# JuliaLinearAlgebra/AlgebraicMultigrid.jl

Hardware: AMD Instinct MI355X
Metric: V-cycle unknowns/sec + fine-level SpMV GB/s (% HBM peak), 3-D Poisson 256^3 (higher is better)
Workload: dtype f64

## Files before the change

algebraicmultigrid.jl_amd/_libs.py:

```python
import ctypes as C
import os

_HERE = os.path.dirname(os.path.abspath(__file__))
SETUP_SO = os.path.join(_HERE, "libamgsetup.so")
HIP_SO = os.path.join(_HERE, "libamghip.so")
HIP_F32_SO = os.path.join(_HERE, "libamghip_f32.so")

i32p = C.POINTER(C.c_int32)
f64p = C.POINTER(C.c_double)
i64 = C.c_int64
vp = C.c_void_p


class AMGError(RuntimeError):
    pass


class amgs_options(C.Structure):
    _fields_ = [("theta", C.c_double), ("max_levels", C.c_int32), ("max_coarse", C.c_int32),
                ("hermitian", C.c_int32), ("sa_omega", C.c_double), ("sa_improve_iters", C.c_int32),
                ("sa_B_is_vector", C.c_int32)]


class amgh_smoother_t(C.Structure):
# ... 141 lines not shown
    L.amgh_dev_upload.argtypes = [C.c_int, vp, vp, i64]
    L.amgh_dev_download.argtypes = [C.c_int, vp, vp, i64]
    L.amgh_dev_sync.argtypes = [C.c_int]
    L.amgh_stream.restype = vp
    L.amgh_stream.argtypes = [vp]
    L.amgh_timer_begin.argtypes = [vp]
    L.amgh_timer_end.argtypes = [vp, C.POINTER(C.c_double)]
    L.amgh_bench_op.argtypes = [vp, C.c_int, C.c_int, C.c_int, C.c_int, C.POINTER(C.c_double)]
    L.amgh_debug_chain_timing.argtypes = [C.c_int, vp]
    L.amgh_debug_merged_sweep_host.argtypes = [i64, i64, vp, vp, vp, C.c_int, C.c_int, C.c_double, vp, vp]
    L.amgh_debug_bw_poll_giveups.argtypes = [vp, C.c_int]
    L.amgh_debug_bw_mode.argtypes = [vp, C.c_int]
    L.amgh_debug_bw_dict.argtypes = [vp, C.c_int]
    L.amgh_debug_bw_late.argtypes = [vp, C.c_int]
    L.amgh_debug_coded_ops.argtypes = [vp, C.c_int]
    L.amgh_debug_bw_sweep_host.argtypes = [i64, vp, vp, vp, C.c_int, C.c_int, C.c_double, vp, vp, vp]
    L.amgh_debug_bw_dict_sweep_host.argtypes = [i64, vp, vp, vp, C.c_int, C.c_int, vp, vp, vp]
    L.amgh_debug_set_tunable.argtypes = [C.c_char_p, C.c_int]
    L.amgh_debug_get_tunable.argtypes = [C.c_char_p, C.POINTER(C.c_int)]
    L.amgh_profile_enable.argtypes = [vp, C.c_int]
    L.amgh_profile_read.argtypes = [vp, vp, C.c_int]
    L.amgh_set_use_graph.argtypes = [vp, C.c_int]


def _bind_dist(L):
    i64p = C.POINTER(i64)
    L.amgh_dist_rccl_available.argtypes = []
    L.amgh_dist_unique_id.argtypes = [vp]
    L.amgh_dist_create_rccl.argtypes = [C.POINTER(vp), C.c_int, C.c_int, C.c_int, vp]
    L.amgh_local_group_create.argtypes = [C.POINTER(vp), C.c_int]
# ... 101 lines not shown
```

algebraicmultigrid.jl_amd/csrc/hip/amghip.hip:

```cpp
#include "amghip_internal.hpp"
#include "gs_schedule.hpp"
#include "csr_ops.hpp"
#include "chebyshev.hpp"
#include "gmres_kernels.hpp"
#include "pcg_block_kernels.hpp"
#include "dist_pcg_kernels.hpp"

namespace {

constexpr int64_t kGraphAutoRows = 65536;

struct Level {
  int64_t n = 0, nc = 0;
  amgh_csr A, S, P, R;
  bool has_S = false;
  amgh_smoother_t pre{}, post{};
  real *res = nullptr, *cx = nullptr, *cb = nullptr, *tmp = nullptr;
  real* cheb_d = nullptr;
  ChebSide cheb[2];
  const ChebSide& cheb_of(const amgh_smoother_t& s) const { return &s == &post ? cheb[1] : cheb[0]; }
  real* il = nullptr;
  amgh_csr* smat() { return has_S ? &S : &A; }
  amgh_csr Pp, Rp;
  bool lo_ok = false;
  real* lo_val = nullptr;
  CodedCols lo_cc;
  bool r_stream = false, p_stream = false;
  bool lo_want = false;
  bool coarse_lo = false;
};

}

struct amgh_handle {
  int device = 0;
  int nrhs = 1;
  hipStream_t stream = nullptr;
  hipStream_t own_stream = nullptr;
  bool ext_stream = false;
  std::vector<Level*> levels;
// ... 202 lines not shown
  {
    ProfScope p(h, AMGH_T_PRESMOOTH, l);
    RC_TRY(smooth(h, L, L->pre, xc, xo, b, bs, xzero,  lo_io,  lo_io && !xzero,  lo));
  }
  if (lo) {
    Level* C = (L->coarse_lo && l + 1 < (int)h->levels.size()) ? h->levels[l + 1] : nullptr;
    GsSchedule* cg = C ? C->smat()->gs : nullptr;
    if (C && !(cg && C->lo_ok && cg->nblk == 0 && cg->cols_alloc >= bs)) return AMGH_ESTATE;
    const int64_t xs = g->xstride;
    {
      ProfScope p(h, AMGH_T_RESIDUAL, l);
      if (il_block(bs) && g_rhs_il >= 2)
        RC_TRY(resid_cols(bs, g->rowptr, g->col, L->lo_val ? L->lo_val : g->val, n, g->xp, xs, g->bp, n, L->res, n, h->stream, &L->lo_cc));
      else
        RC_TRY(raw_apply(M_RESID, g->rowptr, g->col, L->lo_val ? L->lo_val : g->val, n, g->xp, xs, g->bp, n, L->res, n,
                         h->stream, bs, &L->lo_cc));
    }
    {
      ProfScope p(h, AMGH_T_RESTRICT, l);
      if (L->il && il_block(bs) && !(L->r_stream && g_rhs_il == 1))
        RC_TRY(il_apply(bs, false, L->Rp.rowptr, L->Rp.col, L->Rp.val, nc, L->res, n, n, L->il, C ? cg->bp : L->cb, nc, h->stream, &L->Rp.cc));
      else
        RC_TRY(csr_apply(&L->Rp, M_SPMV, L->res, nullptr, C ? cg->bp : L->cb, h->stream, bs));
      if (C) cg->bp_cols = bs;
    }
    if (!C) RC_TRY(vec_fill(h, L->cx, nc * bs, 0.0));
    if (l == (int)h->levels.size() - 1) {
      ProfScope p(h, AMGH_T_COARSE, l + 1);
      for (int c = 0; c < bs; ++c) RC_TRY(coarse_solve(h, L->cx + c * nc, L->cb + c * nc));
    } else if (tail_here(h, l + 1, cyc) && (C != nullptr) == h->tail_lo) {
      ProfScope p(h, AMGH_T_COARSE, l + 1);
      RC_TRY(tail_apply(h, h->tail[cyc].M, nc, C ? cg->xp : L->cx, C ? cg->xstride : nc, C ? (const real*)cg->bp : (const real*)L->cb, nc, bs, false));
    } else {
      RC_TRY(cycle_next(h, l + 1, L->cx, L->cb, cyc, C != nullptr));
    }
    {
      ProfScope p(h, AMGH_T_PROLONG, l);
      if (L->il && il_block(bs) && !(L->p_stream && g_rhs_il == 1))
        RC_TRY(il_apply(bs, true, L->Pp.rowptr, L->Pp.col, L->Pp.val, n, C ? cg->xp : L->cx, nc, C ? cg->xstride : nc, L->il,
                        g->xp, xs, h->stream, &L->Pp.cc));
      else
        RC_TRY(raw_apply(M_ADD, L->Pp.rowptr, L->Pp.col, L->Pp.val, n, C ? cg->xp : L->cx, C ? cg->xstride : nc, nullptr, 0, g->xp,
                         xs, h->stream, bs, &L->Pp.cc));
    }
    {
      ProfScope p(h, AMGH_T_POSTSMOOTH, l);
      RC_TRY(smooth(h, L, L->post, xc, xo, b, bs, false, true, true,  lo_io));
    }
    return AMGH_OK;
  }
  {
    ProfScope p(h, AMGH_T_RESIDUAL, l);
    RC_TRY(csr_apply(&L->A, M_RESID, xc, b, L->res, h->stream, bs));
  }
  {
    ProfScope p(h, AMGH_T_RESTRICT, l);
    if (L->il && il_block(bs))
      RC_TRY(il_apply(bs, false, L->R.rowptr, L->R.col, L->R.val, nc, L->res, n, n, L->il, L->cb, nc, h->stream));
    else
      RC_TRY(csr_apply(&L->R, M_SPMV, L->res, nullptr, L->cb, h->stream, bs));
  }
  RC_TRY(vec_fill(h, L->cx, nc * bs, 0.0));
  if (l == (int)h->levels.size() - 1) {
    ProfScope p(h, AMGH_T_COARSE, l + 1);
    for (int c = 0; c < bs; ++c) RC_TRY(coarse_solve(h, L->cx + c * nc, L->cb + c * nc));
  } else if (tail_here(h, l + 1, cyc) && !h->tail_lo) {
    ProfScope p(h, AMGH_T_COARSE, l + 1);
    RC_TRY(tail_apply(h, h->tail[cyc].M, nc, L->cx, nc, L->cb, nc, bs, false));
  } else {
    RC_TRY(cycle_next(h, l + 1, L->cx, L->cb, cyc));
  }
  {
    ProfScope p(h, AMGH_T_PROLONG, l);
    if (L->il && il_block(bs))
      RC_TRY(il_apply(bs, true, L->P.rowptr, L->P.col, L->P.val, n, L->cx, nc, nc, L->il, xc, n, h->stream));
    else
      RC_TRY(csr_apply(&L->P, M_ADD, L->cx, nullptr, xc, h->stream, bs));
  }
  {
    ProfScope p(h, AMGH_T_POSTSMOOTH, l);
    const bool b_kept = (L->pre.kind == AMGH_SMOOTH_GS || L->pre.kind == AMGH_SMOOTH_SOR) && L->pre.iter > 0;
    RC_TRY(smooth(h, L, L->post, xc, xo, b, bs, false, b_kept));
  }
  if (xc != x) RC_TRY(vec_copy(h, x, xc, n * bs));
  return AMGH_OK;
}

int apply_once(amgh_t* h, real* x, const real* b, int cyc, bool xzero) {
  if (h->levels.empty()) {
    ProfScope p(h, AMGH_T_COARSE, 0);
    for (int c = 0; c < h->nrhs; ++c) RC_TRY(coarse_solve(h, x + c * h->ncoarse, b + c * h->ncoarse));
    return AMGH_OK;
// ... 479 lines not shown
  *hp = h;
  return AMGH_OK;
}

static void level_discard(Level* L);

void amgh_destroy(amgh_t* h) {
  if (!h) return;
  hipSetDevice(h->device);
  if (h->stream) hipStreamSynchronize(h->stream);
  if (h->pending_level) level_discard(h->pending_level);
  for (Level* L : h->levels) {
    csr_free(&L->A); csr_free(&L->S); csr_free(&L->P); csr_free(&L->R); csr_free(&L->Pp); csr_free(&L->Rp);
    hipFree(L->res); hipFree(L->cx); hipFree(L->cb); hipFree(L->tmp); hipFree(L->cheb_d); hipFree(L->lo_val); hipFree(L->il);
    L->lo_cc.free_dev();
    delete L;
  }
  csr_free(&h->finalA);
  hipFree(h->coarse_op); hipFree(h->res_final); hipFree(h->partial); hipFree(h->scal);
  hipFree(h->x0); hipFree(h->b0); hipFree(h->pc_r); hipFree(h->pc_c); hipFree(h->pc_u);
  hipFree(h->gm_V); hipFree(h->gm_t); hipFree(h->gm_sc); hipFree(h->gm_part); hipFree(h->gm_flags);
  hipFree(h->pb_r); hipFree(h->pb_c); hipFree(h->pb_u); hipFree(h->pb_part); hipFree(h->pb_sc); hipFree(h->pb_st);
  for (auto& t : h->tail) hipFree(t.M);
  for (auto& e : h->pending) { hipEventDestroy(e.a); hipEventDestroy(e.b); }
  for (auto& g : h->graphs) if (g.exec) hipGraphExecDestroy(g.exec);
  if (h->t0) hipEventDestroy(h->t0);
  if (h->t1) hipEventDestroy(h->t1);
  if (h->tb0) hipEventDestroy(h->tb0);
  if (h->tb1) hipEventDestroy(h->tb1);
  if (h->own_stream) hipStreamDestroy(h->own_stream);
  else if (h->stream) hipStreamDestroy(h->stream);
  delete h;
}

static void level_discard(Level* L) {
  csr_free(&L->A); csr_free(&L->S); csr_free(&L->P); csr_free(&L->R); csr_free(&L->Pp); csr_free(&L->Rp);
  hipFree(L->lo_val);
  L->lo_cc.free_dev();
  delete L;
}

namespace {
__global__ void perm_rowlen_kernel(const int32_t* rowptr, const int32_t* perm, int64_t n, int32_t* len) {
  const int64_t p = (int64_t)blockIdx.x * blockDim.x + threadIdx.x;
  if (p < n) len[p] = rowptr[perm[p] + 1] - rowptr[perm[p]];
}
__global__ void perm_rows_kernel(const int32_t* rowptr, const int32_t* col, const real* val, const int32_t* perm,
                                 const int32_t* new_rowptr, int64_t n, int32_t* ncol, real* nval) {
  const int ln = threadIdx.x % kWave;
  const int64_t waves = (int64_t)gridDim.x * (blockDim.x / kWave);
  for (int64_t p = (int64_t)blockIdx.x * (blockDim.x / kWave) + threadIdx.x / kWave; p < n; p += waves) {
    const int32_t src = rowptr[perm[p]], len = rowptr[perm[p] + 1] - src, dst = new_rowptr[p];
    for (int e = ln; e < len; e += kWave) { ncol[dst + e] = col[src + e]; nval[dst + e] = val[src + e]; }
// ... 465 lines not shown
      for (int v = 0; v < 2 && rc == AMGH_OK; ++v) {
        L->Rp.xcd_map = v == 1;
        rc = csr_apply(&L->Rp, M_SPMV, L->res, nullptr, L->cb, h->stream, 1);
        if (rc == AMGH_OK && hipEventRecord(h->t0, h->stream) != hipSuccess) rc = -1001;
        for (int r = 0; r < 4 && rc == AMGH_OK; ++r) rc = csr_apply(&L->Rp, M_SPMV, L->res, nullptr, L->cb, h->stream, 1);
        float t = 0.f;
        if (rc == AMGH_OK && (hipEventRecord(h->t1, h->stream) != hipSuccess || hipEventSynchronize(h->t1) != hipSuccess ||
                              hipEventElapsedTime(&t, h->t0, h->t1) != hipSuccess)) rc = -1001;
        ms[v] = t;
      }
      L->Rp.xcd_map = false;
      RC_TRY(rc);
      L->Rp.xcd_map = ms[1] < 0.93 * ms[0];
      if (getenv("AMGH_VERBOSE")) fprintf(stderr, "[amghip] n=%lld restriction: %.3f ms, XCD-contiguous %.3f ms -> %s\n", (long long)L->n, ms[0] / 4, ms[1] / 4, L->Rp.xcd_map ? "XCD-contiguous" : "plain");
    }
  if (gs_trim() && g_stream_code && g_trim_coded) {
    HIP_TRY(hipStreamSynchronize(h->stream));
    for (Level* L : h->levels) {
      for (amgh_csr* M : {&L->Rp, &L->Pp})
        if (M->cc.ccol && M->col && M->val) {
          hipFree(M->col); hipFree(M->val); M->col = nullptr; M->val = nullptr;
          M->bytes -= M->nnz * kEntB;
        }
      amgh_csr* S = L->smat();
      GsSchedule* g = S->gs;
      if (L->lo_cc.ccol && g && g->bw.on && g->bw.flow.on && !g->bw.rec && g->segs.empty() && !g->mf && !g->mb && g->col && g->val) {
        hipFree(g->col); hipFree(g->val); g->col = nullptr; g->val = nullptr;
        int64_t freed = g->nnz * kEntB;
        if (L->lo_val) { hipFree(L->lo_val); L->lo_val = nullptr; }
        g->csr_bytes -= freed; g->bytes -= freed; S->bytes -= freed;
// ... 354 lines not shown
  amgh_csr* op = nullptr;
  switch (which) {
    case AMGH_OP_A: op = &h->levels[level]->A; break;
    case AMGH_OP_P: op = &h->levels[level]->P; break;
    case AMGH_OP_R: op = &h->levels[level]->R; break;
  }
  return (op && op->rowptr) ? op : nullptr;
}

struct LoOp {
  const int32_t *rowptr = nullptr, *col = nullptr;
  const real* val = nullptr;
  int64_t nrows = 0, ncols = 0;
  const int32_t *row_perm = nullptr, *col_perm = nullptr;
  const CodedCols* cc = nullptr;
};
static bool level_lo_op(amgh_t* h, int level, int which, LoOp* o) {
  if (level < 0 || level >= (int)h->levels.size()) return false;
  Level* L = h->levels[level];
  GsSchedule* g = L->smat()->gs;
  if (!L->lo_ok || !g || !g->perm) return false;
  const int32_t* coarse_perm = nullptr;
  if (L->coarse_lo) {
    if (level + 1 >= (int)h->levels.size()) return false;
    GsSchedule* cg = h->levels[level + 1]->smat()->gs;
    if (!cg || !cg->perm) return false;
    coarse_perm = cg->perm;
  }
  switch (which) {
    case AMGH_OP_A:
      if ((int64_t)g->ncols != L->n) return false;
      *o = LoOp{g->rowptr, g->col, L->lo_val ? L->lo_val : g->val, L->n, L->n, g->perm, g->perm, &L->lo_cc};
      return g->rowptr != nullptr && !g->compacted;
    case AMGH_OP_P:
      *o = LoOp{L->Pp.rowptr, L->Pp.col, L->Pp.val, L->n, L->nc, g->perm, coarse_perm, &L->Pp.cc};
      return L->Pp.rowptr != nullptr;
    case AMGH_OP_R:
      *o = LoOp{L->Rp.rowptr, L->Rp.col, L->Rp.val, L->nc, L->n, coarse_perm, g->perm, &L->Rp.cc};
      return L->Rp.rowptr != nullptr;
  }
  return false;
}

static int level_apply(amgh_t* h, int level, int which, int mode, const real* x_d, const real* b_d, real* y_d) {
  if (amgh_csr* op = level_op(h, level, which)) return csr_apply(op, mode, x_d, b_d, y_d, h->stream);
  LoOp o;
  if (!level_lo_op(h, level, which, &o)) return AMGH_EINVAL;
  real *xi = nullptr, *yo = nullptr, *bi = nullptr;
  int rc = AMGH_OK;
  const real* xin = x_d;
  const real* bin = b_d;
  if (o.col_perm) {
    rc = dev_alloc(&xi, o.ncols);
// ... 272 lines not shown
      z ^= z >> 31;
      hx[i] = (real)(z >> 11) * (1.0 / 9007199254740992.0);
    }
    hipMemcpy(x, hx.data(), sizeof(real) * nx, hipMemcpyHostToDevice);
    hipMemcpy(b, hx.data(), sizeof(real) * nx, hipMemcpyHostToDevice);
    hipMemcpy(y, hx.data(), sizeof(real) * nx, hipMemcpyHostToDevice);
  }
  int rc = AMGH_OK;
  auto run = [&]() -> int {
    if (which == 4) {
      if (level >= (int)h->levels.size()) return AMGH_EINVAL;
      return level_smooth_enqueue(h, level, 0, y, b);
    }
    const int mode = (which == 3 || which == 5) ? M_RESID : M_SPMV;
    if (op) return csr_apply(op, mode, x, b, y, h->stream);
    return raw_apply(mode, lo.rowptr, lo.col, lo.val, lo.nrows, x, lo.ncols, b, lo.nrows, y, lo.nrows, h->stream, 1, lo.cc);
    if (which == 4) {
      if (level >= (int)h->levels.size()) return AMGH_EINVAL;
      return level_smooth_enqueue(h, level, 0, y, b);
    }
    return AMGH_EINVAL;
  };
  for (int i = 0; i < warmup && rc == AMGH_OK; ++i) rc = run();
  if (rc == AMGH_OK) {
    hipEventRecord(h->tb0, h->stream);
    for (int i = 0; i < reps && rc == AMGH_OK; ++i) rc = run();
    hipEventRecord(h->tb1, h->stream);
    hipEventSynchronize(h->tb1);
    float f = 0.f;
    hipEventElapsedTime(&f, h->tb0, h->tb1);
    *avg_ms = (double)f / reps;
// ... 308 lines not shown
  else if (!strcmp(name, "gs_bigslot")) *value = g_gs_bigslot;
  else if (!strcmp(name, "gs_super")) *value = g_gs_super;
  else if (!strcmp(name, "gs_block_pipe")) *value = g_gs_block_pipe;
  else return AMGH_EINVAL;
  return AMGH_OK;
}

int amgh_debug_set_perm_io(int on) {
  g_gs_flow_perm_io = on != 0;
  ++g_sched_epoch;
  return AMGH_OK;
}
int amgh_debug_get_perm_io(void) { return g_gs_flow_perm_io; }
int amgh_debug_perm_io_sweeps(int which) { return (which == 0 || which == 1) ? (int)(g_perm_io_sweeps[which] & 0x7fffffffu) : -1; }

int amgh_debug_chain_timing(int enable, unsigned long long* out8) {
  if (enable && !g_chain_tim) {
    HIP_TRY(hipMalloc((void**)&g_chain_tim, 8 * sizeof(unsigned long long)));
    HIP_TRY(hipMemset(g_chain_tim, 0, 8 * sizeof(unsigned long long)));
  }
  if (out8 && g_chain_tim) {
    HIP_TRY(hipDeviceSynchronize());
    HIP_TRY(hipMemcpy(out8, g_chain_tim, 8 * sizeof(unsigned long long), hipMemcpyDeviceToHost));
    HIP_TRY(hipMemset(g_chain_tim, 0, 8 * sizeof(unsigned long long)));
  }
  if (!enable && g_chain_tim) { hipFree(g_chain_tim); g_chain_tim = nullptr; }
  return AMGH_OK;
}

int amgh_profile_enable(amgh_t* h, int on) {
// ... 27 lines not shown
```

algebraicmultigrid.jl_amd/csrc/hip/amghip_internal.hpp:

```cpp
#pragma once
#include "amghip_kernels.hpp"
#include "gs_blocks.hpp"
#include "gs_flow.hpp"

#include <algorithm>
#include <chrono>
#include <cmath>
#include <cstdio>
#include <cstring>
#include <atomic>
#include <mutex>
#include <string>
#include <system_error>
#include <thread>
#include <utility>
#include <vector>

#include "../../../include/amghip.h"

using namespace amgh;

#define HIP_TRY(expr)                                   \
  do {                                                  \
    hipError_t e_ = (expr);                             \
// ... 286 lines not shown
    hipFree(rowmeta); hipFree(desc); hipFree(bp); hipFree(xp); hipFree(permx);
    d_lvl_ptr = rowptr = col = perm = dpos = nullptr; val = diag = bp = xp = nullptr; rowmeta = desc = nullptr; permx = nullptr;
  }
};

}

#include "dev_scan.hpp"

struct CodedCols {
  uint32_t* ccol = nullptr; real* vtab = nullptr; int n = 0;
  int64_t bytes = 0;
  void free_dev() { hipFree(ccol); hipFree(vtab); ccol = nullptr; vtab = nullptr; n = 0; bytes = 0; }
};

struct amgh_csr {
  CodedCols cc;
  bool cc_tried = false;
  bool xcd_map = false;
  int device = 0;
  int64_t nrows = 0, ncols = 0, nnz = 0;
  int32_t* rowptr = nullptr;
  int32_t* col = nullptr;
  real* val = nullptr;
  int32_t* dpos = nullptr;
  real* diag = nullptr;
  GsSchedule* gs = nullptr;
  int gs_nrhs_hint = 0;
  uint32_t pipe_epoch = 0; const void* pipe_rmbox = nullptr; int pipe_grid = 0;
  int64_t bytes = 0;
};

// ... 11 lines not shown
int g_gs_bw = 1;
int g_gs_bw_rows = 512;
int g_gs_bw_flow = 1;
int g_gs_bw_spin = 0;
int g_gs_bw_skip_pub = -1;
int g_gs_bw_nc = -1;
int g_gs_bw_nrhs = 1;
int g_gs_bw_chain = 1;
int g_stream_code = 1;
int g_trim_coded = 1;
int g_gs_bw_inorder = 0;
int g_gs_bw_dict = 1;
int g_gs_bw_relay = 3;
int g_gs_flow_xzero = 1;
int g_gs_flow_perm_io = 1;
unsigned int g_perm_io_sweeps[2] = {0, 0};
int g_gs_bw_two_min_rows = 200000;
int g_gs_sell = 1;
int g_gs_lean = -1;
int g_gs_ept = 0;
int g_gs_lpr = 0;
int g_gs_il = 1;
int g_pcg_fused = 1;
int g_tail_dense_rows = 6144;
int g_tail_dense = 1;
int g_gs_dense_blk = 4096;
int g_gs_dense_tri = 1;
int g_gs_block_inverse = 1;

std::atomic<unsigned long long> g_sched_epoch{0};
// ... 25 lines not shown
  op->nrows = nrows;
  op->ncols = ncols;
  op->nnz = nnz;
  RC_TRY(dev_upload(&op->rowptr, rowptr, nrows + 1));
  RC_TRY(dev_upload(&op->col, col, nnz));
  RC_TRY(dev_upload(&op->val, val, nnz));
  op->bytes = (nrows + 1) * 4 + nnz * kEntB;
  return AMGH_OK;
}

void csr_free(amgh_csr* op) {
  if (!op) return;
  hipFree(op->rowptr); hipFree(op->col); hipFree(op->val);
  hipFree(op->dpos); hipFree(op->diag);
  op->cc.free_dev();
  if (op->gs) { op->gs->free_dev(); delete op->gs; }
  op->rowptr = op->col = op->dpos = nullptr; op->val = op->diag = nullptr; op->gs = nullptr;
}

int csr_ensure_diag(amgh_csr* op, hipStream_t st) {
  if (op->dpos) return AMGH_OK;
  const int64_t n = std::min(op->nrows, op->ncols);
  RC_TRY(dev_alloc(&op->dpos, op->nrows));
  RC_TRY(dev_alloc(&op->diag, op->nrows));
  if (n < op->nrows) {
    HIP_TRY(hipMemsetAsync(op->dpos, 0xff, sizeof(int32_t) * op->nrows, st));
    HIP_TRY(hipMemsetAsync(op->diag, 0, sizeof(real) * op->nrows, st));
  }
  if (n > 0)
    hipLaunchKernelGGL(find_diag_kernel, dim3((unsigned)((n + 255) / 256)), dim3(256), 0, st, op->rowptr, op->col,
// ... 9 lines not shown
```

algebraicmultigrid.jl_amd/csrc/hip/amghip_kernels.hpp:

```cpp
#pragma once
#include <hip/hip_runtime.h>
#include <stdint.h>

#ifndef AMGH_REAL
#define AMGH_REAL double
#endif

namespace amgh {

using real = AMGH_REAL;

constexpr int kWave = 64;
constexpr int kThreads = 256;
constexpr int kNumXcd = 8;

enum StreamMode : int {
  M_SPMV = 0,
  M_RESID = 1,
  M_ADD = 2,
  M_JACOBI = 3,
  M_GS = 4,
  M_SOR = 5,
  M_CHEB1 = 6,
  M_CHEB = 7
// ... 246 lines not shown
    } else {
      const int i = gi[q];
      const real d = gd[q];
      if (d != 0.0) {
        if (MODE == M_GS) {
          a.y[i] = (gb[q] - acc[q]) / d;
        } else {
          a.y[i] = (1.0 - a.omega) * a.y[i] + (a.omega / d) * (gb[q] - acc[q]);
        }
      }
    }
  }
}

using DefaultCfg = StreamCfg<1024, 1024, 8192, 4, false, false>;

__device__ __forceinline__ real seq_sum_range(const real* s, int lo, int hi, real acc) {
  int j = lo;
  if (hi - j >= 8) {
    real p[8], q[8];
#pragma unroll
    for (int e = 0; e < 8; ++e) p[e] = s[j + e];
    j += 8;
    while (hi - j >= 16) {
#pragma unroll
      for (int e = 0; e < 8; ++e) q[e] = s[j + e];
#pragma unroll
      for (int e = 0; e < 8; ++e) acc += p[e];
#pragma unroll
      for (int e = 0; e < 8; ++e) p[e] = s[j + 8 + e];
// ... 1658 lines not shown
```

algebraicmultigrid.jl_amd/csrc/hip/csr_ops.hpp:

```cpp
#pragma once
#include <atomic>

namespace {


template <int MODE, class CFG = DefaultCfg, bool CODED = false>
int launch_stream(const StreamArgs& a0, hipStream_t st, int ncolv = 1) {
  const int nrows = a0.row_end - a0.row_begin;
  if (nrows <= 0) return AMGH_OK;
  StreamArgs a = a0;
  a.ncolv = ncolv;
  const int nb = (nrows + CFG::ROWS - 1) / CFG::ROWS;
  const int64_t grid = (CFG::XCD || ncolv > 1) ? (int64_t)((nb + kNumXcd - 1) / kNumXcd) * kNumXcd * ncolv : nb;
  hipLaunchKernelGGL((csr_stream_kernel<MODE, CFG, CODED>), dim3((unsigned)grid), dim3(CFG::THREADS), 0, st, a);
  HIP_TRY(hipGetLastError());
  return AMGH_OK;
}

constexpr int kGsBlockTarget = 256;
constexpr int kGsMinRows = 4;
constexpr int kGsNnzPerWg = 256;
template <int MODE>
int launch_gs_level(const StreamArgs& a, int rows, hipStream_t st, int ncolv = 1) {
  const int width = a.row_end - a.row_begin;
// ... 45 lines not shown
  for (int64_t k = (int64_t)blockIdx.x * blockDim.x + threadIdx.x; k < nnz; k += (int64_t)gridDim.x * blockDim.x) {
    const real v = val[k];
    if (code_find(s_tab, ntab, real_bits(v)) >= 0) continue;
    if (__hip_atomic_load(miss_cnt, __ATOMIC_RELAXED, __HIP_MEMORY_SCOPE_AGENT) >= (unsigned)kCodeMiss) continue;
    const unsigned i = atomicAdd(miss_cnt, 1u);
    if (i < (unsigned)kCodeMiss) miss[i] = v;
  }
}
__global__ void code_encode_kernel(const int32_t* col, const real* val, int64_t nnz, const real* tab, int ntab, uint32_t* ccol) {
  __shared__ rbits_t s_tab[kCodeMax];
  if ((int)threadIdx.x < ntab) s_tab[threadIdx.x] = real_bits(tab[threadIdx.x]);
  __syncthreads();
  for (int64_t k = (int64_t)blockIdx.x * blockDim.x + threadIdx.x; k < nnz; k += (int64_t)gridDim.x * blockDim.x)
    ccol[k] = (uint32_t)col[k] | ((uint32_t)code_find(s_tab, ntab, real_bits(val[k])) << kCodeBits);
}
int code_values(const int32_t* col, const real* val, int64_t nrows, int64_t ncols, int64_t nnz, CodedCols* out, hipStream_t st) {
  if (!g_stream_code || out->ccol || nrows < (1 << 18) || ncols > ((int64_t)1 << kCodeBits) || nnz <= 0 || !col || !val) return AMGH_OK;
  unsigned* d_cnt = nullptr; real *d_miss = nullptr, *d_tab = nullptr;
  RC_TRY(dev_alloc(&d_cnt, 1));
  int rc = dev_alloc(&d_miss, kCodeMiss);
  if (rc == AMGH_OK) rc = dev_alloc(&d_tab, kCodeMax);
  std::vector<rbits_t> tab;
  std::vector<real> miss((size_t)kCodeMiss);
  bool ok = rc == AMGH_OK;
  for (int pass = 0; ok && pass < 8; ++pass) {
    const int64_t span = pass == 0 ? std::min<int64_t>(nnz, 1 << 20) : nnz;
    const int ntab = (int)tab.size();
    if (hipMemsetAsync(d_cnt, 0, 4, st) != hipSuccess) { rc = -1001; break; }
    if (ntab > 0) {
      std::vector<real> tv((size_t)ntab);
      for (int i = 0; i < ntab; ++i) std::memcpy(&tv[(size_t)i], &tab[(size_t)i], sizeof(real));
      if (hipMemcpyAsync(d_tab, tv.data(), sizeof(real) * (size_t)ntab, hipMemcpyHostToDevice, st) != hipSuccess) { rc = -1001; break; }
// ... 18 lines not shown
    if (rc == AMGH_OK) rc = dev_alloc(&out->vtab, kCodeMax);
    if (rc == AMGH_OK && hipMemcpyAsync(d_tab, tv.data(), sizeof(real) * tv.size(), hipMemcpyHostToDevice, st) != hipSuccess) rc = -1001;
    if (rc == AMGH_OK && hipMemcpyAsync(out->vtab, tv.data(), sizeof(real) * tv.size(), hipMemcpyHostToDevice, st) != hipSuccess) rc = -1001;
    if (rc == AMGH_OK) {
      hipLaunchKernelGGL(code_encode_kernel, dim3((unsigned)std::min<int64_t>((nnz + 255) / 256, 8192)), dim3(256), 0, st, col, val, nnz, (const real*)d_tab, (int)tab.size(), out->ccol);
      if (hipGetLastError() != hipSuccess || hipStreamSynchronize(st) != hipSuccess) rc = -1001;
    }
    if (rc == AMGH_OK) { out->n = (int)tab.size(); out->bytes = nnz * 4 + kCodeMax * kRealB; }
    else out->free_dev();
  }
  hipFree(d_cnt); hipFree(d_miss); hipFree(d_tab);
  if (rc == AMGH_ENOMEM) { (void)hipGetLastError(); out->free_dev(); return AMGH_OK; }
  return rc;
}

int csr_apply(const amgh_csr* op, int mode, const real* x, const real* b, real* y, hipStream_t st,
              int ncolv = 1) {
  StreamArgs a{};
  a.rowptr = op->rowptr; a.col = op->col; a.val = op->val;
  a.ccol = op->cc.ccol; a.vtab = op->cc.vtab; a.vtab_n = op->cc.n;
  a.x = x; a.y = y; a.b = b;
  a.row_begin = 0; a.row_end = (int32_t)op->nrows;
  a.ldx = op->ncols; a.ldy = op->nrows; a.ldb = op->nrows;
  switch (mode) {
    case M_SPMV: return launch_stream_sized<M_SPMV>(a, st, ncolv, op->xcd_map);
    case M_RESID: return launch_stream_sized<M_RESID>(a, st, ncolv);
    case M_ADD: return launch_stream_sized<M_ADD>(a, st, ncolv);
  }
  return AMGH_EINVAL;
}

int csr_jacobi(amgh_csr* op, real omega, const real* xin, const real* b, real* xout, hipStream_t st,
               int ncolv = 1) {
  RC_TRY(csr_ensure_diag(op, st));
  StreamArgs a{};
  a.rowptr = op->rowptr; a.col = op->col; a.val = op->val;
  a.x = xin; a.y = xout; a.b = b; a.dpos = op->dpos; a.diag = op->diag; a.omega = omega;
  a.row_begin = 0; a.row_end = (int32_t)op->nrows;
// ... 126 lines not shown
  switch (threads) {
    case 64: return launch_chain_tiny_t<64>(c, sor, n, nnz, nlev, st, ncolv);
    case 256: return launch_chain_tiny_t<256>(c, sor, n, nnz, nlev, st, ncolv);
    default: return launch_chain_tiny_t<1024>(c, sor, n, nnz, nlev, st, ncolv);
  }
}
int launch_chain(const ChainArgs& c, bool sor, bool ldsx, int threads, int nx, hipStream_t st, int ncolv) {
  switch (threads) {
    case 64: return launch_chain_t<64, 4>(c, sor, ldsx, nx, st, ncolv);
    case 256: return launch_chain_t<256, 4>(c, sor, ldsx, nx, st, ncolv);
    default: return launch_chain_t<1024, 4>(c, sor, ldsx, nx, st, ncolv);
  }
}

int raw_apply(int mode, const int32_t* rowptr, const int32_t* col, const real* val, int64_t nrows, const real* x,
              int64_t ldx, const real* b, int64_t ldb, real* y, int64_t ldy, hipStream_t st, int ncolv, const CodedCols* cc = nullptr) {
  StreamArgs a{};
  a.rowptr = rowptr; a.col = col; a.val = val;
  if (cc) { a.ccol = cc->ccol; a.vtab = cc->vtab; a.vtab_n = cc->n; }
  a.x = x; a.y = y; a.b = b;
  a.row_begin = 0; a.row_end = (int32_t)nrows;
  a.ldx = ldx; a.ldy = ldy; a.ldb = ldb;
  switch (mode) {
    case M_SPMV: return launch_stream_sized<M_SPMV>(a, st, ncolv);
    case M_RESID: return launch_stream_sized<M_RESID>(a, st, ncolv);
    case M_ADD: return launch_stream_sized<M_ADD>(a, st, ncolv);
  }
  return AMGH_EINVAL;
}

template <int BS>
int il_apply_t(bool add, const int32_t* rowptr, const int32_t* col, const real* val, int64_t nrows, const real* x, int64_t nx,
               int64_t ldx, real* il, real* y, int64_t ldy, hipStream_t st, const CodedCols* cc) {
  if (nx > 0)
    hipLaunchKernelGGL((to_interleaved_kernel<BS>), dim3((unsigned)((nx + 63) / 64)), dim3(256), 0, st, x, ldx, il, nx);
  const int64_t threads = nrows * BS;
  if (threads > 0) {
// ... 545 lines not shown
```

include/amghip.h:

```cpp
#ifndef AMGHIP_H
#define AMGHIP_H

#include <stdint.h>

#ifdef __cplusplus
extern "C" {
#endif

#ifndef AMGH_REAL
#define AMGH_REAL double
#endif
typedef AMGH_REAL amgh_real;

typedef struct amgh_handle amgh_t;
typedef struct amgh_csr amgh_csr_t;

#define AMGH_OK 0
#define AMGH_EINVAL (-2)
#define AMGH_ESTATE (-3)
#define AMGH_ENOMEM (-4)
#define AMGH_EUNSUPPORTED (-5)

enum { AMGH_SMOOTH_NONE = 0, AMGH_SMOOTH_GS = 1, AMGH_SMOOTH_JACOBI = 2, AMGH_SMOOTH_SOR = 3, AMGH_SMOOTH_CHEBYSHEV = 4 };
enum { AMGH_SWEEP_FORWARD = 0, AMGH_SWEEP_BACKWARD = 1, AMGH_SWEEP_SYMMETRIC = 2 };
// ... 219 lines not shown
int amgh_debug_bw_dict_sweep_host(int64_t nrows, const int32_t* rowptr, const int32_t* col, const amgh_real* val, int target_rows,
                                  int backward, amgh_real* x, const amgh_real* b, int64_t* stats5);

int amgh_debug_bw_poll_giveups(const amgh_t* h, int l);

int amgh_debug_bw_mode(const amgh_t* h, int l);
int amgh_debug_bw_dict(const amgh_t* h, int l);
int amgh_debug_bw_late(const amgh_t* h, int l);
int amgh_debug_coded_ops(const amgh_t* h, int l);

int amgh_debug_set_tunable(const char* name, int value);
int amgh_debug_get_tunable(const char* name, int* value);
int amgh_debug_set_perm_io(int on);
int amgh_debug_get_perm_io(void);
int amgh_debug_perm_io_sweeps(int which);

int amgh_set_use_graph(amgh_t* h, int on);

#ifdef __cplusplus
}
#endif
#endif
```

Before: 1.212 billion.

## Add sliced-ELL SpMV path for residual, restriction and prolongation with autotuned selection

```diff
diff --git a/algebraicmultigrid.jl_amd/_libs.py b/algebraicmultigrid.jl_amd/_libs.py
--- a/algebraicmultigrid.jl_amd/_libs.py
+++ b/algebraicmultigrid.jl_amd/_libs.py
@@ -179,6 +179,14 @@
     L.amgh_debug_bw_dict.argtypes = [vp, C.c_int]
     L.amgh_debug_bw_late.argtypes = [vp, C.c_int]
     L.amgh_debug_coded_ops.argtypes = [vp, C.c_int]
+    L.amgh_debug_set_sell_stream.argtypes = [C.c_int, i64, C.c_int]
+    L.amgh_debug_sell_stream_launches.argtypes = [vp, C.c_int, C.c_int]
+    L.amgh_debug_sell_stream_padded.argtypes = [vp, C.c_int, C.c_int]
+    L.amgh_debug_sell_stream_padded.restype = i64
+    L.amgh_debug_csr_sell.argtypes = [vp, C.c_int]
+    L.amgh_debug_csr_sell.restype = i64
+    L.amgh_debug_csr_sell_launches.argtypes = [vp]
+    L.amgh_debug_csr_sell_apply.argtypes = [vp, C.c_int, vp, vp, vp]
     L.amgh_debug_bw_sweep_host.argtypes = [i64, vp, vp, vp, C.c_int, C.c_int, C.c_double, vp, vp, vp]
     L.amgh_debug_bw_dict_sweep_host.argtypes = [i64, vp, vp, vp, C.c_int, C.c_int, vp, vp, vp]
     L.amgh_debug_set_tunable.argtypes = [C.c_char_p, C.c_int]
diff --git a/algebraicmultigrid.jl_amd/csrc/hip/amghip.hip b/algebraicmultigrid.jl_amd/csrc/hip/amghip.hip
--- a/algebraicmultigrid.jl_amd/csrc/hip/amghip.hip
+++ b/algebraicmultigrid.jl_amd/csrc/hip/amghip.hip
@@ -24,6 +24,7 @@
   amgh_csr Pp, Rp;
   bool lo_ok = false;
   real* lo_val = nullptr;
+  SellCols lo_sc;
   CodedCols lo_cc;
   bool r_stream = false, p_stream = false;
   bool lo_want = false;
@@ -256,14 +257,14 @@
         RC_TRY(resid_cols(bs, g->rowptr, g->col, L->lo_val ? L->lo_val : g->val, n, g->xp, xs, g->bp, n, L->res, n, h->stream, &L->lo_cc));
       else
         RC_TRY(raw_apply(M_RESID, g->rowptr, g->col, L->lo_val ? L->lo_val : g->val, n, g->xp, xs, g->bp, n, L->res, n,
-                         h->stream, bs, &L->lo_cc));
+                         h->stream, bs, &L->lo_cc, &L->lo_sc));
     }
     {
       ProfScope p(h, AMGH_T_RESTRICT, l);
       if (L->il && il_block(bs) && !(L->r_stream && g_rhs_il == 1))
         RC_TRY(il_apply(bs, false, L->Rp.rowptr, L->Rp.col, L->Rp.val, nc, L->res, n, n, L->il, C ? cg->bp : L->cb, nc, h->stream, &L->Rp.cc));
       else
-        RC_TRY(csr_apply(&L->Rp, M_SPMV, L->res, nullptr, C ? cg->bp : L->cb, h->stream, bs));
+        RC_TRY(csr_apply(&L->Rp, M_SPMV, L->res, nullptr, C ? cg->bp : L->cb, h->stream, bs, true));
       if (C) cg->bp_cols = bs;
     }
     if (!C) RC_TRY(vec_fill(h, L->cx, nc * bs, 0.0));
@@ -283,7 +284,7 @@
                         g->xp, xs, h->stream, &L->Pp.cc));
       else
         RC_TRY(raw_apply(M_ADD, L->Pp.rowptr, L->Pp.col, L->Pp.val, n, C ? cg->xp : L->cx, C ? cg->xstride : nc, nullptr, 0, g->xp,
-                         xs, h->stream, bs, &L->Pp.cc));
+                         xs, h->stream, bs, &L->Pp.cc, &L->Pp.sc));
     }
     {
       ProfScope p(h, AMGH_T_POSTSMOOTH, l);
@@ -293,14 +294,14 @@
   }
   {
     ProfScope p(h, AMGH_T_RESIDUAL, l);
-    RC_TRY(csr_apply(&L->A, M_RESID, xc, b, L->res, h->stream, bs));
+    RC_TRY(csr_apply(&L->A, M_RESID, xc, b, L->res, h->stream, bs, true));
   }
   {
     ProfScope p(h, AMGH_T_RESTRICT, l);
     if (L->il && il_block(bs))
       RC_TRY(il_apply(bs, false, L->R.rowptr, L->R.col, L->R.val, nc, L->res, n, n, L->il, L->cb, nc, h->stream));
     else
-      RC_TRY(csr_apply(&L->R, M_SPMV, L->res, nullptr, L->cb, h->stream, bs));
+      RC_TRY(csr_apply(&L->R, M_SPMV, L->res, nullptr, L->cb, h->stream, bs, true));
   }
   RC_TRY(vec_fill(h, L->cx, nc * bs, 0.0));
   if (l == (int)h->levels.size() - 1) {
@@ -317,7 +318,7 @@
     if (L->il && il_block(bs))
       RC_TRY(il_apply(bs, true, L->P.rowptr, L->P.col, L->P.val, n, L->cx, nc, nc, L->il, xc, n, h->stream));
     else
-      RC_TRY(csr_apply(&L->P, M_ADD, L->cx, nullptr, xc, h->stream, bs));
+      RC_TRY(csr_apply(&L->P, M_ADD, L->cx, nullptr, xc, h->stream, bs, true));
   }
   {
     ProfScope p(h, AMGH_T_POSTSMOOTH, l);
@@ -827,6 +828,7 @@
     csr_free(&L->A); csr_free(&L->S); csr_free(&L->P); csr_free(&L->R); csr_free(&L->Pp); csr_free(&L->Rp);
     hipFree(L->res); hipFree(L->cx); hipFree(L->cb); hipFree(L->tmp); hipFree(L->cheb_d); hipFree(L->lo_val); hipFree(L->il);
     L->lo_cc.free_dev();
+    L->lo_sc.free_dev();
     delete L;
   }
   csr_free(&h->finalA);
@@ -850,6 +852,7 @@
   csr_free(&L->A); csr_free(&L->S); csr_free(&L->P); csr_free(&L->R); csr_free(&L->Pp); csr_free(&L->Rp);
   hipFree(L->lo_val);
   L->lo_cc.free_dev();
+  L->lo_sc.free_dev();
   delete L;
 }
 
@@ -1345,6 +1348,61 @@
       L->Rp.xcd_map = ms[1] < 0.93 * ms[0];
       if (getenv("AMGH_VERBOSE")) fprintf(stderr, "[amghip] n=%lld restriction: %.3f ms, XCD-contiguous %.3f ms -> %s\n", (long long)L->n, ms[0] / 4, ms[1] / 4, L->Rp.xcd_map ? "XCD-contiguous" : "plain");
     }
+  if (h->nrhs == 1)
+    for (Level* L : h->levels) {
+      GsSchedule* g = L->smat()->gs;
+      const bool cd = g_stream_code != 0;
+      if (!(L->lo_ok && g && g->nblk == 0)) {
+        for (amgh_csr* M : {&L->A, &L->R, &L->P})
+          if (M->rowptr) { RC_TRY(sell_build(M->rowptr, cd ? M->cc.ccol : nullptr, M->col, M->val, M->nrows, M->nnz, &M->sc, h->stream)); ws += M->sc.bytes; }
+        continue;
+      }
+      if (!g->rowptr || g->compacted) continue;
+      RC_TRY(sell_build(g->rowptr, cd ? L->lo_cc.ccol : nullptr, g->col, L->lo_val ? L->lo_val : g->val, L->n, g->nnz, &L->lo_sc, h->stream));
+      RC_TRY(sell_build(L->Rp.rowptr, cd ? L->Rp.cc.ccol : nullptr, L->Rp.col, L->Rp.val, L->Rp.nrows, L->Rp.nnz, &L->Rp.sc, h->stream));
+      RC_TRY(sell_build(L->Pp.rowptr, cd ? L->Pp.cc.ccol : nullptr, L->Pp.col, L->Pp.val, L->Pp.nrows, L->Pp.nnz, &L->Pp.sc, h->stream));
+      if (L->n >= (1 << 18) && g_sell_min_rows >= ((int64_t)1 << 18)) {
+        real* ty = nullptr;
+        RC_TRY(dev_alloc(&ty, L->n));
+        int rc = AMGH_OK;
+        if (hipMemsetAsync(ty, 0, sizeof(real) * L->n, h->stream) != hipSuccess || hipMemsetAsync(L->res, 0, sizeof(real) * L->n, h->stream) != hipSuccess ||
+            hipMemsetAsync(L->cx, 0, sizeof(real) * L->nc, h->stream) != hipSuccess) rc = -1001;
+        const real* val = L->lo_val ? L->lo_val : g->val;
+        auto run = [&](int which) -> int {
+          if (which == AMGH_OP_A) return raw_apply(M_RESID, g->rowptr, g->col, val, L->n, L->res, L->n, L->res, L->n, ty, L->n, h->stream, 1, &L->lo_cc, &L->lo_sc);
+          if (which == AMGH_OP_R) return csr_apply(&L->Rp, M_SPMV, L->res, nullptr, L->cb, h->stream, 1, true);
+          return raw_apply(M_ADD, L->Pp.rowptr, L->Pp.col, L->Pp.val, L->n, L->cx, L->nc, nullptr, 0, ty, L->n, h->stream, 1, &L->Pp.cc, &L->Pp.sc);
+        };
+        const int keep = g_sell_stream;
+        for (int which : {AMGH_OP_A, AMGH_OP_R, AMGH_OP_P}) {
+          SellCols* sc = which == AMGH_OP_A ? &L->lo_sc : which == AMGH_OP_R ? &L->Rp.sc : &L->Pp.sc;
+          if (!sc->w || (which == AMGH_OP_R ? L->Rp.nrows : L->n) < (1 << 18)) continue;
+          double ms[2] = {0, 0};
+          for (int v = 0; v < 2 && rc == AMGH_OK; ++v) {
+            g_sell_stream = v;
+            rc = run(which);
+            if (rc == AMGH_OK && hipEventRecord(h->t0, h->stream) != hipSuccess) rc = -1001;
+            for (int r = 0; r < 4 && rc == AMGH_OK; ++r) rc = run(which);
+            float t = 0.f;
+            if (rc == AMGH_OK && (hipEventRecord(h->t1, h->stream) != hipSuccess || hipEventSynchronize(h->t1) != hipSuccess ||
+                                  hipEventElapsedTime(&t, h->t0, h->t1) != hipSuccess)) rc = -1001;
+            ms[v] = t;
+          }
+          sc->launches = 0;
+          if (rc != AMGH_OK) break;
+          if (getenv("AMGH_VERBOSE")) fprintf(stderr, "[amghip] n=%lld operator %d: csr_stream_kernel %.3f ms, sliced-ELL %.3f ms\n", (long long)L->n, which, ms[0] / 4, ms[1] / 4);
+          if (!(ms[1] < 0.97 * ms[0])) sc->free_dev();
+        }
+        g_sell_stream = keep;
+        if (hipStreamSynchronize(h->stream) != hipSuccess && rc == AMGH_OK) rc = -1001;
+        hipFree(ty);
+        RC_TRY(rc);
+      }
+      ws += L->lo_sc.bytes + L->Rp.sc.bytes + L->Pp.sc.bytes;
+      if (getenv("AMGH_VERBOSE"))
+        fprintf(stderr, "[amghip] n=%lld sliced-ELL padded / entries: A %.3f  R %.3f  P %.3f (0: not taken)\n", (long long)L->n, (double)L->lo_sc.padded / std::max<int64_t>(1, g->nnz),
+                (double)L->Rp.sc.padded / std::max<int64_t>(1, L->Rp.nnz), (double)L->Pp.sc.padded / std::max<int64_t>(1, L->Pp.nnz));
+    }
   if (gs_trim() && g_stream_code && g_trim_coded) {
     HIP_TRY(hipStreamSynchronize(h->stream));
     for (Level* L : h->levels) {
@@ -1729,6 +1787,7 @@
   int64_t nrows = 0, ncols = 0;
   const int32_t *row_perm = nullptr, *col_perm = nullptr;
   const CodedCols* cc = nullptr;
+  const SellCols* sc = nullptr;
 };
 static bool level_lo_op(amgh_t* h, int level, int which, LoOp* o) {
   if (level < 0 || level >= (int)h->levels.size()) return false;
@@ -1745,13 +1804,13 @@
   switch (which) {
     case AMGH_OP_A:
       if ((int64_t)g->ncols != L->n) return false;
-      *o = LoOp{g->rowptr, g->col, L->lo_val ? L->lo_val : g->val, L->n, L->n, g->perm, g->perm, &L->lo_cc};
+      *o = LoOp{g->rowptr, g->col, L->lo_val ? L->lo_val : g->val, L->n, L->n, g->perm, g->perm, &L->lo_cc, &L->lo_sc};
       return g->rowptr != nullptr && !g->compacted;
     case AMGH_OP_P:
-      *o = LoOp{L->Pp.rowptr, L->Pp.col, L->Pp.val, L->n, L->nc, g->perm, coarse_perm, &L->Pp.cc};
+      *o = LoOp{L->Pp.rowptr, L->Pp.col, L->Pp.val, L->n, L->nc, g->perm, coarse_perm, &L->Pp.cc, &L->Pp.sc};
       return L->Pp.rowptr != nullptr;
     case AMGH_OP_R:
-      *o = LoOp{L->Rp.rowptr, L->Rp.col, L->Rp.val, L->nc, L->n, coarse_perm, g->perm, &L->Rp.cc};
+      *o = LoOp{L->Rp.rowptr, L->Rp.col, L->Rp.val, L->nc, L->n, coarse_perm, g->perm, &L->Rp.cc, &L->Rp.sc};
       return L->Rp.rowptr != nullptr;
   }
   return false;
@@ -2054,7 +2113,7 @@
     }
     const int mode = (which == 3 || which == 5) ? M_RESID : M_SPMV;
     if (op) return csr_apply(op, mode, x, b, y, h->stream);
-    return raw_apply(mode, lo.rowptr, lo.col, lo.val, lo.nrows, x, lo.ncols, b, lo.nrows, y, lo.nrows, h->stream, 1, lo.cc);
+    return raw_apply(mode, lo.rowptr, lo.col, lo.val, lo.nrows, x, lo.ncols, b, lo.nrows, y, lo.nrows, h->stream, 1, lo.cc, which >= 5 ? lo.sc : nullptr);
     if (which == 4) {
       if (level >= (int)h->levels.size()) return AMGH_EINVAL;
       return level_smooth_enqueue(h, level, 0, y, b);
@@ -2393,6 +2452,51 @@
 int amgh_debug_get_perm_io(void) { return g_gs_flow_perm_io; }
 int amgh_debug_perm_io_sweeps(int which) { return (which == 0 || which == 1) ? (int)(g_perm_io_sweeps[which] & 0x7fffffffu) : -1; }
 
+int amgh_debug_set_sell_stream(int on, int64_t min_rows, int cap_pct) {
+  g_sell_stream = on != 0;
+  g_sell_min_rows = min_rows > 0 ? min_rows : (int64_t)1 << 18;
+  g_sell_cap_pct = cap_pct > 0 ? cap_pct : 0;
+  ++g_sched_epoch;
+  return AMGH_OK;
+}
+int amgh_debug_get_sell_stream(void) { return g_sell_stream; }
+static const SellCols* sell_of(const amgh_t* h, int level, int which) {
+  if (!h || level < 0 || level >= (int)h->levels.size()) return nullptr;
+  const Level* L = h->levels[level];
+  const GsSchedule* g = (L->has_S ? L->S : L->A).gs;
+  if (!(L->lo_ok && g && g->nblk == 0))
+    return which == AMGH_OP_A ? &L->A.sc : which == AMGH_OP_R ? &L->R.sc : which == AMGH_OP_P ? &L->P.sc : nullptr;
+  return which == AMGH_OP_A ? &L->lo_sc : which == AMGH_OP_R ? &L->Rp.sc : which == AMGH_OP_P ? &L->Pp.sc : nullptr;
+}
+int amgh_debug_sell_stream_launches(const amgh_t* h, int level, int which) {
+  const SellCols* sc = sell_of(h, level, which);
+  return sc ? (int)(sc->launches & 0x7fffffffu) : -1;
+}
+int64_t amgh_debug_sell_stream_padded(const amgh_t* h, int level, int which) {
+  const SellCols* sc = sell_of(h, level, which);
+  return sc ? (sc->w ? sc->padded : 0) : -1;
+}
+
+int64_t amgh_debug_csr_sell(amgh_csr_t* op, int coded) {
+  if (!op) return AMGH_EINVAL;
+  HIP_TRY(hipSetDevice(op->device));
+  if (coded && !op->cc.ccol) {
+    RC_TRY(code_values(op->col, op->val, op->nrows, op->ncols, op->nnz, &op->cc, nullptr, 1));
+    op->bytes += op->cc.bytes;
+  }
+  RC_TRY(sell_build(op->rowptr, coded ? op->cc.ccol : nullptr, op->col, op->val, op->nrows, op->nnz, &op->sc, nullptr));
+  op->bytes += op->sc.bytes;
+  return op->sc.w ? op->sc.padded : 0;
+}
+int amgh_debug_csr_sell_apply(amgh_csr_t* op, int mode, const real* x_d, const real* b_d, real* y_d) {
+  if (!op || !x_d || !y_d || mode < M_SPMV || mode > M_ADD || (mode == M_RESID && !b_d)) return AMGH_EINVAL;
+  HIP_TRY(hipSetDevice(op->device));
+  RC_TRY(csr_apply(op, mode, x_d, b_d, y_d, nullptr, 1, true));
+  HIP_TRY(hipDeviceSynchronize());
+  return AMGH_OK;
+}
+int amgh_debug_csr_sell_launches(const amgh_csr_t* op) { return op ? (int)(op->sc.launches & 0x7fffffffu) : -1; }
+
 int amgh_debug_chain_timing(int enable, unsigned long long* out8) {
   if (enable && !g_chain_tim) {
     HIP_TRY(hipMalloc((void**)&g_chain_tim, 8 * sizeof(unsigned long long)));
diff --git a/algebraicmultigrid.jl_amd/csrc/hip/amghip_internal.hpp b/algebraicmultigrid.jl_amd/csrc/hip/amghip_internal.hpp
--- a/algebraicmultigrid.jl_amd/csrc/hip/amghip_internal.hpp
+++ b/algebraicmultigrid.jl_amd/csrc/hip/amghip_internal.hpp
@@ -324,8 +324,18 @@
   void free_dev() { hipFree(ccol); hipFree(vtab); ccol = nullptr; vtab = nullptr; n = 0; bytes = 0; }
 };
 
+constexpr int kSellCapPct = 130, kSellCapPlainPct = 110;
+constexpr int kSellLongSteps = 12;
+struct SellCols {
+  uint32_t* w = nullptr; real* v = nullptr; uint2* slice = nullptr; uint8_t* len8 = nullptr;
+  int64_t nslices = 0, padded = 0, bytes = 0;
+  unsigned launches = 0;
+  void free_dev() { hipFree(w); hipFree(v); hipFree(slice); hipFree(len8); w = nullptr; v = nullptr; slice = nullptr; len8 = nullptr; nslices = padded = bytes = 0; }
+};
+
 struct amgh_csr {
   CodedCols cc;
+  SellCols sc;
   bool cc_tried = false;
   bool xcd_map = false;
   int device = 0;
@@ -367,6 +377,9 @@
 int g_gs_bw_relay = 3;
 int g_gs_flow_xzero = 1;
 int g_gs_flow_perm_io = 1;
+int g_sell_stream = 1;
+int64_t g_sell_min_rows = (int64_t)1 << 18;
+int g_sell_cap_pct = 0;
 unsigned int g_perm_io_sweeps[2] = {0, 0};
 int g_gs_bw_two_min_rows = 200000;
 int g_gs_sell = 1;
@@ -422,6 +435,7 @@
   hipFree(op->rowptr); hipFree(op->col); hipFree(op->val);
   hipFree(op->dpos); hipFree(op->diag);
   op->cc.free_dev();
+  op->sc.free_dev();
   if (op->gs) { op->gs->free_dev(); delete op->gs; }
   op->rowptr = op->col = op->dpos = nullptr; op->val = op->diag = nullptr; op->gs = nullptr;
 }
diff --git a/algebraicmultigrid.jl_amd/csrc/hip/amghip_kernels.hpp b/algebraicmultigrid.jl_amd/csrc/hip/amghip_kernels.hpp
--- a/algebraicmultigrid.jl_amd/csrc/hip/amghip_kernels.hpp
+++ b/algebraicmultigrid.jl_amd/csrc/hip/amghip_kernels.hpp
@@ -284,6 +284,95 @@
 }
 
 using DefaultCfg = StreamCfg<1024, 1024, 8192, 4, false, false>;
+
+struct SellStreamArgs {
+  const uint32_t* w;
+  const real* v;
+  const uint2* slice;
+  const uint8_t* len;
+  const int32_t* rowptr;
+  const real* vtab;
+  int32_t vtab_n;
+  int32_t nrows, nslices;
+  const real* x;
+  const real* b;
+  real* y;
+};
+template <int MODE, bool CODED, int B>
+__global__ __launch_bounds__(kThreads) void sell_stream_kernel(SellStreamArgs a) {
+  static_assert(MODE == M_SPMV || MODE == M_RESID || MODE == M_ADD, "SpMV-type passes only");
+  __shared__ real s_tab[CODED ? kCodeMax : 1];
+  if (CODED) {
+    if ((int)threadIdx.x < a.vtab_n) s_tab[threadIdx.x] = a.vtab[threadIdx.x];
+    __syncthreads();
+  }
+  const int s = (int)blockIdx.x * (kThreads / kWave) + __builtin_amdgcn_readfirstlane((int)(threadIdx.x >> 6));
+  if (s >= a.nslices) return;
+  const int lane = threadIdx.x & (kWave - 1);
+  const int r = s * kWave + lane;
+  const bool live = r < a.nrows;
+  int len = 0;
+  if (live) len = a.len ? (int)a.len[r] : a.rowptr[r + 1] - a.rowptr[r];
+  const uint2 sd = a.slice[s];
+  const int nit = (int)sd.y;
+  const int64_t base = (int64_t)sd.x * kWave + lane;
+  uint32_t w[B];
+  real v[B];
+#pragma unroll
+  for (int e = 0; e < B; ++e) {
+    w[e] = 0; v[e] = 0.0;
+    if (e < nit) { w[e] = a.w[base + (int64_t)e * kWave]; if (!CODED) v[e] = a.v[base + (int64_t)e * kWave]; }
+  }
+  real acc = 0.0;
+  for (int t = 0; t < nit; t += B) {
+    uint32_t wn[B];
+    real vn[B];
+#pragma unroll
+    for (int e = 0; e < B; ++e) {
+      wn[e] = 0; vn[e] = 0.0;
+      if (t + B + e < nit) { wn[e] = a.w[base + (int64_t)(t + B + e) * kWave]; if (!CODED) vn[e] = a.v[base + (int64_t)(t + B + e) * kWave]; }
+    }
+    real xv[B];
+#pragma unroll
+    for (int e = 0; e < B; ++e) {
+      const uint32_t c = CODED ? (w[e] & ((1u << kCodeBits) - 1)) : w[e];
+      xv[e] = t + e < len ? a.x[c] : (real)0.0;
+      if (CODED) v[e] = s_tab[w[e] >> kCodeBits];
+    }
+#pragma unroll
+    for (int e = 0; e < B; ++e)
+      if (t + e < len) acc = acc + v[e] * xv[e];
+#pragma unroll
+    for (int e = 0; e < B; ++e) { w[e] = wn[e]; v[e] = vn[e]; }
+  }
+  if (!live) return;
+  if (MODE == M_SPMV) a.y[r] = acc;
+  else if (MODE == M_RESID) a.y[r] = a.b[r] - acc;
+  else a.y[r] = a.y[r] + acc;
+}
+__global__ void sell_steps_kernel(const int32_t* rowptr, int nrows, int nslices, int32_t* steps) {
+  const int s = blockIdx.x * blockDim.x + threadIdx.x;
+  if (s >= nslices) return;
+  const int r1 = min(s * kWave + kWave, nrows);
+  int m = 0;
+  for (int r = s * kWave; r < r1; ++r) m = max(m, rowptr[r + 1] - rowptr[r]);
+  steps[s] = m;
+}
+__global__ void sell_stream_fill_kernel(const int32_t* rowptr, const uint32_t* w_in, const real* v_in, const uint2* slice, int nrows,
+                                        int nslices, uint32_t* w, real* v, uint8_t* len8) {
+  const int64_t gid = (int64_t)blockIdx.x * blockDim.x + threadIdx.x;
+  const int s = (int)(gid >> 6), lane = (int)(gid & 63);
+  if (s >= nslices) return;
+  const uint2 sd = slice[s];
+  const int r = s * kWave + lane;
+  int32_t a0 = 0, len = 0;
+  if (r < nrows) { a0 = rowptr[r]; len = rowptr[r + 1] - a0; if (len8) len8[r] = (uint8_t)len; }
+  const int64_t base = (int64_t)sd.x * kWave + lane;
+  for (int t = 0; t < (int)sd.y; ++t) {
+    w[base + (int64_t)t * kWave] = t < len ? w_in[a0 + t] : 0u;
+    if (v) v[base + (int64_t)t * kWave] = t < len ? v_in[a0 + t] : (real)0.0;
+  }
+}
 
 __device__ __forceinline__ real seq_sum_range(const real* s, int lo, int hi, real acc) {
   int j = lo;
diff --git a/algebraicmultigrid.jl_amd/csrc/hip/csr_ops.hpp b/algebraicmultigrid.jl_amd/csrc/hip/csr_ops.hpp
--- a/algebraicmultigrid.jl_amd/csrc/hip/csr_ops.hpp
+++ b/algebraicmultigrid.jl_amd/csrc/hip/csr_ops.hpp
@@ -83,8 +83,9 @@
   for (int64_t k = (int64_t)blockIdx.x * blockDim.x + threadIdx.x; k < nnz; k += (int64_t)gridDim.x * blockDim.x)
     ccol[k] = (uint32_t)col[k] | ((uint32_t)code_find(s_tab, ntab, real_bits(val[k])) << kCodeBits);
 }
-int code_values(const int32_t* col, const real* val, int64_t nrows, int64_t ncols, int64_t nnz, CodedCols* out, hipStream_t st) {
-  if (!g_stream_code || out->ccol || nrows < (1 << 18) || ncols > ((int64_t)1 << kCodeBits) || nnz <= 0 || !col || !val) return AMGH_OK;
+int code_values(const int32_t* col, const real* val, int64_t nrows, int64_t ncols, int64_t nnz, CodedCols* out, hipStream_t st,
+                int64_t min_rows = (int64_t)1 << 18) {
+  if (!g_stream_code || out->ccol || nrows < min_rows || ncols > ((int64_t)1 << kCodeBits) || nnz <= 0 || !col || !val) return AMGH_OK;
   unsigned* d_cnt = nullptr; real *d_miss = nullptr, *d_tab = nullptr;
   RC_TRY(dev_alloc(&d_cnt, 1));
   int rc = dev_alloc(&d_miss, kCodeMiss);
@@ -133,14 +134,75 @@
   return rc;
 }
 
+int sell_build(const int32_t* rowptr, const uint32_t* ccol, const int32_t* col, const real* val, int64_t nrows, int64_t nnz,
+               SellCols* out, hipStream_t st) {
+  if (out->w || nrows < g_sell_min_rows || nrows <= 0 || nnz <= 0 || !rowptr || (!ccol && !(col && val))) return AMGH_OK;
+  const int64_t ns = (nrows + kWave - 1) / kWave;
+  int32_t* d_steps = nullptr;
+  RC_TRY(dev_alloc(&d_steps, ns));
+  hipLaunchKernelGGL(sell_steps_kernel, dim3((unsigned)((ns + 255) / 256)), dim3(256), 0, st, rowptr, (int)nrows, (int)ns, d_steps);
+  std::vector<int32_t> steps((size_t)ns);
+  if (hipMemcpyAsync(steps.data(), d_steps, sizeof(int32_t) * ns, hipMemcpyDeviceToHost, st) != hipSuccess || hipStreamSynchronize(st) != hipSuccess) { hipFree(d_steps); return -1001; }
+  hipFree(d_steps);
+  std::vector<uint2> sd((size_t)ns);
+  int64_t off = 0;
+  int longest = 0;
+  for (int64_t s = 0; s < ns; ++s) { sd[(size_t)s] = make_uint2((unsigned)off, (unsigned)steps[(size_t)s]); off += steps[(size_t)s]; longest = std::max(longest, steps[(size_t)s]); }
+  const int64_t padded = off * kWave;
+  const bool coded = ccol != nullptr;
+  if (off >= ((int64_t)1 << 32) || padded * 100 > nnz * (int64_t)(g_sell_cap_pct > 0 ? g_sell_cap_pct : coded ? kSellCapPct : kSellCapPlainPct)) return AMGH_OK;
+  int rc = dev_alloc(&out->w, padded);
+  if (rc == AMGH_OK && !coded) rc = dev_alloc(&out->v, padded);
+  if (rc == AMGH_OK) rc = dev_alloc(&out->slice, ns);
+  if (rc == AMGH_OK && longest <= 255) rc = dev_alloc(&out->len8, nrows);
+  if (rc == AMGH_OK && hipMemcpyAsync(out->slice, sd.data(), sizeof(uint2) * ns, hipMemcpyHostToDevice, st) != hipSuccess) rc = -1001;
+  if (rc == AMGH_OK) {
+    hipLaunchKernelGGL(sell_stream_fill_kernel, dim3((unsigned)((ns * kWave + 255) / 256)), dim3(256), 0, st, rowptr,
+                       coded ? ccol : (const uint32_t*)col, coded ? (const real*)nullptr : val, (const uint2*)out->slice, (int)nrows, (int)ns,
+                       out->w, out->v, out->len8);
+    if (hipGetLastError() != hipSuccess || hipStreamSynchronize(st) != hipSuccess) rc = -1001;
+  }
+  if (rc != AMGH_OK) { out->free_dev(); if (rc == AMGH_ENOMEM) { (void)hipGetLastError(); return AMGH_OK; } return rc; }
+  out->nslices = ns; out->padded = padded;
+  out->bytes = padded * (coded ? 4 : kEntB) + ns * 8 + (out->len8 ? nrows : 0);
+  return AMGH_OK;
+}
+bool sell_apply(int mode, const StreamArgs& a, const SellCols* sc, hipStream_t st, int ncolv, int* rc) {
+  if (!sc || !sc->w || !g_sell_stream || ncolv != 1 || (!sc->v && !a.vtab)) return false;
+  SellStreamArgs s{};
+  s.w = sc->w; s.v = sc->v; s.slice = sc->slice; s.len = sc->len8; s.rowptr = a.rowptr; s.vtab = a.vtab; s.vtab_n = a.vtab_n;
+  s.nrows = a.row_end; s.nslices = (int32_t)sc->nslices; s.x = a.x; s.b = a.b; s.y = a.y;
+  const dim3 grid((unsigned)((sc->nslices + kThreads / kWave - 1) / (kThreads / kWave))), block(kThreads);
+  const bool coded = sc->v == nullptr;
+  const bool b8 = coded && sc->padded >= (int64_t)kSellLongSteps * kWave * sc->nslices;
+#define AMGH_SELL_LAUNCH(M) \
+  do { \
+    if (b8) hipLaunchKernelGGL((sell_stream_kernel<M, true, 8>), grid, block, 0, st, s); \
+    else if (coded) hipLaunchKernelGGL((sell_stream_kernel<M, true, 4>), grid, block, 0, st, s); \
+    else hipLaunchKernelGGL((sell_stream_kernel<M, false, 4>), grid, block, 0, st, s); \
+  } while (0)
+  switch (mode) {
+    case M_SPMV: AMGH_SELL_LAUNCH(M_SPMV); break;
+    case M_RESID: AMGH_SELL_LAUNCH(M_RESID); break;
+    case M_ADD: AMGH_SELL_LAUNCH(M_ADD); break;
+    default: return false;
+  }
+#undef AMGH_SELL_LAUNCH
+  ++const_cast<SellCols*>(sc)->launches;
+  *rc = hipGetLastError() == hipSuccess ? AMGH_OK : -1001;
+  return true;
+}
+
 int csr_apply(const amgh_csr* op, int mode, const real* x, const real* b, real* y, hipStream_t st,
-              int ncolv = 1) {
+              int ncolv = 1, bool sell = false) {
   StreamArgs a{};
   a.rowptr = op->rowptr; a.col = op->col; a.val = op->val;
   a.ccol = op->cc.ccol; a.vtab = op->cc.vtab; a.vtab_n = op->cc.n;
   a.x = x; a.y = y; a.b = b;
   a.row_begin = 0; a.row_end = (int32_t)op->nrows;
   a.ldx = op->ncols; a.ldy = op->nrows; a.ldb = op->nrows;
+  int rc = AMGH_OK;
+  if (sell && sell_apply(mode, a, &op->sc, st, ncolv, &rc)) return rc;
   switch (mode) {
     case M_SPMV: return launch_stream_sized<M_SPMV>(a, st, ncolv, op->xcd_map);
     case M_RESID: return launch_stream_sized<M_RESID>(a, st, ncolv);
@@ -297,13 +359,16 @@
 }
 
 int raw_apply(int mode, const int32_t* rowptr, const int32_t* col, const real* val, int64_t nrows, const real* x,
-              int64_t ldx, const real* b, int64_t ldb, real* y, int64_t ldy, hipStream_t st, int ncolv, const CodedCols* cc = nullptr) {
+              int64_t ldx, const real* b, int64_t ldb, real* y, int64_t ldy, hipStream_t st, int ncolv, const CodedCols* cc = nullptr,
+              const SellCols* sc = nullptr) {
   StreamArgs a{};
   a.rowptr = rowptr; a.col = col; a.val = val;
   if (cc) { a.ccol = cc->ccol; a.vtab = cc->vtab; a.vtab_n = cc->n; }
   a.x = x; a.y = y; a.b = b;
   a.row_begin = 0; a.row_end = (int32_t)nrows;
   a.ldx = ldx; a.ldy = ldy; a.ldb = ldb;
+  int rc = AMGH_OK;
+  if (sell_apply(mode, a, sc, st, ncolv, &rc)) return rc;
   switch (mode) {
     case M_SPMV: return launch_stream_sized<M_SPMV>(a, st, ncolv);
     case M_RESID: return launch_stream_sized<M_RESID>(a, st, ncolv);
diff --git a/include/amghip.h b/include/amghip.h
--- a/include/amghip.h
+++ b/include/amghip.h
@@ -257,6 +257,13 @@
 int amgh_debug_set_perm_io(int on);
 int amgh_debug_get_perm_io(void);
 int amgh_debug_perm_io_sweeps(int which);
+int amgh_debug_set_sell_stream(int on, int64_t min_rows, int cap_pct);
+int amgh_debug_get_sell_stream(void);
+int amgh_debug_sell_stream_launches(const amgh_t* h, int level, int which);
+int64_t amgh_debug_sell_stream_padded(const amgh_t* h, int level, int which);
+int64_t amgh_debug_csr_sell(amgh_csr_t* op, int coded);
+int amgh_debug_csr_sell_apply(amgh_csr_t* op, int mode, const amgh_real* x_d, const amgh_real* b_d, amgh_real* y_d);
+int amgh_debug_csr_sell_launches(const amgh_csr_t* op);
 
 int amgh_set_use_graph(amgh_t* h, int on);
 
```

Result: faster. 1.225 billion (median of 6 runs) (+1.1%).
